# ramkp990/Truth_Recommendation_GNN

Hardware: NVIDIA B200
Metric: message-passing edges/s (train step) (higher is better)
Workload: dtype f32

## Files before the change

### include/trg_b200.h

```cpp
#ifndef TRG_B200_H
#define TRG_B200_H

#include <stddef.h>
#include <stdint.h>

#ifdef __cplusplus
extern "C" {
#endif

#define TRG_ABI_VERSION 4

enum { TRG_F32 = 0, TRG_BF16 = 1, TRG_F8E4M3 = 2  };
enum {
  TRG_OK = 0,
  TRG_E_ARG = 1,
  TRG_E_WORKSPACE = 2,
  TRG_E_CUDA = 3,
  TRG_E_UNSUPPORTED = 4
};

int trg_abi_version(void);
const char* trg_last_error(void);
int64_t trg_launch_count(void);

size_t trg_csr_workspace_bytes(int64_t n_edges, int64_t n_key);
int trg_csr_build(const int64_t* other, const int64_t* key, int64_t n_edges, int64_t n_key,
                  int32_t* rowptr , int32_t* col , int32_t* eid ,
                  void* workspace, size_t workspace_bytes, void* stream);

size_t trg_select_range_workspace_bytes(int64_t n);
int trg_select_range(const int64_t* key, const int64_t* other, int64_t n, int64_t lo, int64_t hi,
                     int64_t capacity, int64_t pad_key, int64_t pad_other,
                     int64_t* key_out , int64_t* other_out ,
                     int32_t* count_out , void* workspace, size_t workspace_bytes, void* stream);

typedef struct {
  const int32_t* vrowptr;
  const int32_t* vinfo;
  int64_t n_vrows;
  const int32_t* long_rows;
  const int32_t* long_ptr;
  int64_t n_long;
  float* partial;
} trg_long_rows;

int trg_sage_agg_fwd(const int32_t* rowptr, const int32_t* col, const void* x_src,
                     int64_t n_dst, int32_t feat, int dtype,
                     void* mean_out , float* inv_deg_out ,
                     const trg_long_rows* long_rows , void* stream);

int trg_sage_agg_bwd(const int32_t* rowptr_t, const int32_t* col_t, const float* inv_deg,
                     const void* g_mean, int64_t n_src, int32_t feat, int dtype,
                     void* g_src_out , int out_dtype, int accumulate,
                     const void* relu_of, const trg_long_rows* long_rows ,
                     void* stream);

int trg_gather_wsum(const int32_t* rowptr, const int32_t* col, const int32_t* eid,
                    const float* coef, const float* scale, const void* x,
                    int64_t n_rows, int32_t feat, int dtype, void* out, int out_dtype, int accumulate,
                    const void* relu_of, const trg_long_rows* long_rows , void* stream);

int trg_rows_finish(const void* in, int in_dtype, const float* row_scale, const void* add,
                    const void* relu_of, int64_t n_rows, int32_t feat, int dtype, void* out, void* stream);

int trg_peer_reduce_rows(const void* const* parts, int32_t n_peers, int64_t row0, int in_dtype,
                         const float* row_scale, const void* add, const void* relu_of, int64_t n_rows,
                         int32_t feat, int dtype, void* out, int32_t ctas_per_sm, void* stream);

size_t trg_edge_bce_workspace_bytes(int64_t n_users);
int trg_edge_bce_fwd(const int32_t* rowptr_u, const int32_t* col_p, const int32_t* eid,
                     const int64_t* neg_p, const void* u, const void* p,
                     int64_t n_users, int64_t n_edges, int32_t hidden, int dtype,
                     const float* wbar , float* loss_out,
                     float* c_pos, float* c_neg, void* g_u,
                     void* workspace, size_t workspace_bytes, void* stream);

int trg_edge_anchor_loss(const int32_t* rowptr, const int32_t* col, const int32_t* eid,
                         const void* anchor, const void* gathered, int64_t n_rows,
                         int64_t n_edges_scale, int32_t hidden, int dtype, int label,
                         const float* wbar, float* loss_out, float* coef_out, void* g_anchor,
                         int accumulate, int relu_gate, void* workspace, size_t workspace_bytes,
// ... 64 lines not shown
```

### truth_recommendation_gnn_b200/_lib.py

```python
from __future__ import annotations

import ctypes
import os

import torch

_HERE = os.path.dirname(os.path.abspath(__file__))
LIB_PATH = os.path.join(_HERE, "lib", "libtrg_b200.so")

TRG_F32, TRG_BF16, TRG_F8E4M3 = 0, 1, 2
ABI_VERSION = 4

_vp, _i64, _i32, _sz, _int = ctypes.c_void_p, ctypes.c_int64, ctypes.c_int32, ctypes.c_size_t, ctypes.c_int


class TrgProjTerm(ctypes.Structure):
    _fields_ = [("a", _vp), ("w", _vp), ("k", _i32), ("alpha", ctypes.c_float)]


class TrgLongRows(ctypes.Structure):
    _fields_ = [("vrowptr", _vp), ("vinfo", _vp), ("n_vrows", _i64), ("long_rows", _vp), ("long_ptr", _vp),
                ("n_long", _i64), ("partial", _vp)]


class TrgProjBwdTerm(ctypes.Structure):
    _fields_ = [("w", _vp), ("k", _i32), ("alpha", ctypes.c_float), ("row_scale", _vp), ("d_a", _vp)]


class TrgProjDwTerm(ctypes.Structure):
    _fields_ = [("a", _vp), ("k", _i32), ("alpha", ctypes.c_float), ("d_w", _vp)]


SIGNATURES = {
    "trg_abi_version": (_int, []),
    "trg_last_error": (ctypes.c_char_p, []),
    "trg_launch_count": (_i64, []),
    "trg_csr_workspace_bytes": (_sz, [_i64, _i64]),
    "trg_csr_build": (_int, [_vp, _vp, _i64, _i64, _vp, _vp, _vp, _vp, _sz, _vp]),
    "trg_select_range_workspace_bytes": (_sz, [_i64]),
    "trg_select_range": (_int, [_vp, _vp, _i64, _i64, _i64, _i64, _i64, _i64, _vp, _vp, _vp, _vp, _sz, _vp]),
    "trg_sage_agg_fwd": (_int, [_vp, _vp, _vp, _i64, _i32, _int, _vp, _vp, ctypes.POINTER(TrgLongRows), _vp]),
    "trg_sage_agg_bwd": (_int, [_vp, _vp, _vp, _vp, _i64, _i32, _int, _vp, _int, _int, _vp,
                                ctypes.POINTER(TrgLongRows), _vp]),
    "trg_gather_wsum": (_int, [_vp, _vp, _vp, _vp, _vp, _vp, _i64, _i32, _int, _vp, _int, _int, _vp,
                               ctypes.POINTER(TrgLongRows), _vp]),
    "trg_rows_finish": (_int, [_vp, _int, _vp, _vp, _vp, _i64, _i32, _int, _vp, _vp]),
    "trg_peer_reduce_rows": (_int, [_vp, _i32, _i64, _int, _vp, _vp, _vp, _i64, _i32, _int, _vp, _i32, _vp]),
    "trg_edge_bce_workspace_bytes": (_sz, [_i64]),
    "trg_edge_bce_fwd": (_int, [_vp, _vp, _vp, _vp, _vp, _vp, _i64, _i64, _i32, _int, _vp, _vp,
                                _vp, _vp, _vp, _vp, _sz, _vp]),
    "trg_edge_anchor_loss": (_int, [_vp, _vp, _vp, _vp, _vp, _i64, _i64, _i32, _int, _int, _vp, _vp, _vp,
                                    _vp, _int, _int, _vp, _sz, _vp]),
    "trg_sage_proj_workspace_bytes": (_sz, [_i32, _i32, _int]),
    "trg_sage_proj_fwd": (_int, [ctypes.POINTER(TrgProjTerm), _i32, _vp, _i64, _i32, _int, _int, _vp,
                                 _vp, _sz, _vp]),
    "trg_sage_proj_bwd_input": (_int, [_vp, ctypes.POINTER(TrgProjBwdTerm), _i32, _i64, _i32, _int,
                                       _vp, _sz, _vp]),
    "trg_sage_proj_dw_workspace_bytes": (_sz, []),
    "trg_sage_proj_bwd_weight": (_int, [_vp, ctypes.POINTER(TrgProjDwTerm), _i32, _vp, _i64, _i32, _int,
                                        _vp, _sz, _vp]),
    "trg_score_topk_workspace_bytes": (_sz, [_i64, _i64, _i32, _i32]),
    "trg_score_topk": (_int, [_vp, _vp, _i64, _i64, _i32, _int, _i32, _i64, _vp, _vp, _vp, _sz, _vp]),
    "trg_score_topk_excluding": (_int, [_vp, _vp, _i64, _i64, _i32, _int, _i32, _i64, _vp, _vp, _vp, _vp, _vp,
                                        _vp, _sz, _vp]),
    "trg_topk_merge": (_int, [_vp, _vp, _i64, _i32, _i32, _i32, _vp, _vp, _vp]),
    "trg_rescore_topk_workspace_bytes": (_sz, [_i64, _i32]),
    "trg_rescore_topk": (_int, [_vp, _vp, _i64, _i64, _i32, _int, _vp, _i32, _i64, _i32, _vp, _vp, _vp, _sz,
                                _vp]),
}

_lib = None


class TrgError(RuntimeError):
    pass


def load():
    global _lib
    if _lib is None:
        if not os.path.exists(LIB_PATH):
            raise TrgError(
                f"{LIB_PATH} is missing: build it with `python -m truth_recommendation_gnn_b200.build` "
                "(nvcc, sm_100a). There is no CPU or PyTorch fallback for the hot path.")
        lib = ctypes.CDLL(LIB_PATH)
        for name, (res, args) in SIGNATURES.items():
            fn = getattr(lib, name)
            fn.restype, fn.argtypes = res, args
        if lib.trg_abi_version() != ABI_VERSION:
            raise TrgError("libtrg_b200.so ABI version mismatch; rebuild")
        _lib = lib
# ... 68 lines not shown
```

### truth_recommendation_gnn_b200/csrc/csr_build.cu

```cuda
#include <algorithm>
#include <cstdio>

#include "common.cuh"

namespace trg {
namespace {

constexpr int kThreads = 256;
constexpr int kItems = 16;
constexpr int kTile = kThreads * kItems;
constexpr int kWarps = kThreads / 32;
constexpr int kRadix = 256;

template <int NWARPS>
__device__ __forceinline__ int block_exclusive_scan(int v, int* warp_sums, int& total) {
  const int lane = threadIdx.x & 31, w = threadIdx.x >> 5;
  int inc = v;
#pragma unroll
  for (int o = 1; o < 32; o <<= 1) {
    int t = __shfl_up_sync(0xffffffffu, inc, o);
    if (lane >= o) inc += t;
  }
  if (lane == 31) warp_sums[w] = inc;
  __syncthreads();
// ... 19 lines not shown
  for (int i = 0; i < kItems; ++i) {
    int64_t idx = base + (int64_t)i * kThreads + threadIdx.x;
    if (idx < n) s += in[idx];
  }
  int total;
  block_exclusive_scan<kWarps>(s, warp_sums, total);
  if (threadIdx.x == 0) tile_sums[blockIdx.x] = total;
}

__global__ void __launch_bounds__(1024) scan_tile_offsets(int* __restrict__ tile_sums, int n_tiles) {
  __shared__ int warp_sums[32];
  int carry = 0;
  for (int base = 0; base < n_tiles; base += 1024) {
    int idx = base + threadIdx.x;
    int v = idx < n_tiles ? tile_sums[idx] : 0;
    int total;
    int ex = block_exclusive_scan<32>(v, warp_sums, total);
    if (idx < n_tiles) tile_sums[idx] = carry + ex;
    carry += total;
  }
}

__global__ void __launch_bounds__(kThreads) scan_apply(const int* in, int* out, int64_t n,
                                                       const int* __restrict__ tile_offsets) {
  __shared__ int warp_sums[kWarps];
  const int64_t base = (int64_t)blockIdx.x * kTile + (int64_t)threadIdx.x * kItems;
  int v[kItems];
  int s = 0;
#pragma unroll
  for (int i = 0; i < kItems; ++i) {
    v[i] = (base + i < n) ? in[base + i] : 0;
    s += v[i];
  }
  int total;
  int run = block_exclusive_scan<kWarps>(s, warp_sums, total) + tile_offsets[blockIdx.x];
#pragma unroll
  for (int i = 0; i < kItems; ++i) {
    if (base + i < n) out[base + i] = run;
    run += v[i];
  }
}

int exclusive_scan(const int* in, int* out, int64_t n, int* tile_sums, cudaStream_t st) {
  if (n <= 0) return TRG_OK;
  const int n_tiles = (int)ceil_div<int64_t>(n, kTile);
  scan_tile_sums<<<n_tiles, kThreads, 0, st>>>(in, n, tile_sums);
  scan_tile_offsets<<<1, 1024, 0, st>>>(tile_sums, n_tiles);
  scan_apply<<<n_tiles, kThreads, 0, st>>>(in, out, n, tile_sums);
  count_launch(3);
  TRG_LAUNCH_OK();
  return TRG_OK;
}

__global__ void __launch_bounds__(kThreads) count_keys(const long long* __restrict__ key, int64_t n,
                                                       long long n_key, int* __restrict__ deg) {
  int64_t i = (int64_t)blockIdx.x * blockDim.x + threadIdx.x;
  const int64_t stride = (int64_t)gridDim.x * blockDim.x;
  for (; i < n; i += stride) {
    const long long k = ldg_stream(key + i);
    if ((unsigned long long)k >= (unsigned long long)n_key) {
      printf("trg_csr_build: key %lld at edge %lld is outside [0, %lld)\n", k, (long long)i, n_key);
      __trap();
    }
    atomicAdd(&deg[(int)k], 1);
  }
}


__global__ void __launch_bounds__(kThreads) select_count(const long long* __restrict__ key, int64_t n,
                                                         long long lo, long long hi, int* __restrict__ tile_counts) {
  __shared__ int warp_sums[kWarps];
  const int64_t base = (int64_t)blockIdx.x * kTile;
  int c = 0;
#pragma unroll
  for (int i = 0; i < kItems; ++i) {
    const int64_t idx = base + (int64_t)i * kThreads + threadIdx.x;
    if (idx < n) {
      const long long k = ldg_stream(key + idx);
      c += (k >= lo && k < hi) ? 1 : 0;
    }
  }
  int total;
  block_exclusive_scan<kWarps>(c, warp_sums, total);
  if (threadIdx.x == 0) tile_counts[blockIdx.x] = total;
}

__global__ void __launch_bounds__(1024) select_offsets(int* __restrict__ tile_counts, int n_tiles,
                                                       long long capacity, int* __restrict__ count_out) {
  __shared__ int warp_sums[32];
  int carry = 0;
  for (int base = 0; base < n_tiles; base += 1024) {
    const int idx = base + threadIdx.x;
    const int v = idx < n_tiles ? tile_counts[idx] : 0;
    int total;
    const int ex = block_exclusive_scan<32>(v, warp_sums, total);
    if (idx < n_tiles) tile_counts[idx] = carry + ex;
    carry += total;
  }
  if (threadIdx.x == 0) {
    *count_out = carry;
    if ((long long)carry > capacity) {
      printf("trg_select_range: %d selected entries exceed the capacity %lld (negatives far from uniform? pass a larger "
             "capacity)\n", carry, capacity);
      __trap();
    }
  }
}

__global__ void __launch_bounds__(kThreads)
    select_scatter(const long long* __restrict__ key, const long long* __restrict__ other, int64_t n, long long lo,
                   long long hi, const int* __restrict__ tile_offsets, const int* __restrict__ count,
                   long long capacity, long long pad_key, long long pad_other, long long* __restrict__ key_out,
                   long long* __restrict__ other_out) {
  __shared__ int wtot[kWarps];
  const int lane = threadIdx.x & 31, w = threadIdx.x >> 5;
  const int64_t wbase = (int64_t)blockIdx.x * kTile + (int64_t)w * (kItems * 32);
  long long kv[kItems];
  unsigned sel[kItems];
  int mine = 0;
#pragma unroll
  for (int r = 0; r < kItems; ++r) {
    const int64_t idx = wbase + r * 32 + lane;
    kv[r] = idx < n ? ldg_stream(key + idx) : lo - 1;
    const bool in = kv[r] >= lo && kv[r] < hi;
    sel[r] = __ballot_sync(0xffffffffu, in);
    mine += __popc(sel[r]);
  }
  if (lane == 0) wtot[w] = mine;
  __syncthreads();
  int run = tile_offsets[blockIdx.x];
  for (int i = 0; i < w; ++i) run += wtot[i];
#pragma unroll
  for (int r = 0; r < kItems; ++r) {
    if ((sel[r] >> lane) & 1u) {
      const int dest = run + __popc(sel[r] & ((1u << lane) - 1u));
      if (dest < capacity) {
        key_out[dest] = kv[r] - lo;
        other_out[dest] = ldg_stream(other + wbase + r * 32 + lane);
      }
    }
    run += __popc(sel[r]);
  }
  const long long cnt = *count;
  for (long long i = cnt + (long long)blockIdx.x * kThreads + threadIdx.x; i < capacity;
       i += (long long)gridDim.x * kThreads) {
    key_out[i] = pad_key;
    other_out[i] = pad_other;
  }
}

__device__ __forceinline__ uint2 ldg_pair(const uint2* p) {
  uint2 r;
  asm volatile("ld.global.nc.L1::no_allocate.v2.u32 {%0,%1}, [%2];" : "=r"(r.x), "=r"(r.y) : "l"(p));
  return r;
}
template <bool FIRST>
__device__ __forceinline__ uint32_t load_key(const void* keys, int64_t idx) {
  if (FIRST) return (uint32_t)ldg_stream(reinterpret_cast<const long long*>(keys) + idx);
  return ldg_pair(reinterpret_cast<const uint2*>(keys) + idx).x;
}

template <bool FIRST>
__global__ void __launch_bounds__(kThreads) radix_hist(const void* __restrict__ keys, int64_t n,
                                                       int shift, int* __restrict__ hist,
                                                       int n_ctas) {
  __shared__ int h[kRadix];
  h[threadIdx.x] = 0;
  __syncthreads();
  const int64_t base = (int64_t)blockIdx.x * kTile;
#pragma unroll
  for (int i = 0; i < kItems; ++i) {
    int64_t idx = base + (int64_t)i * kThreads + threadIdx.x;
    if (idx < n) atomicAdd(&h[(load_key<FIRST>(keys, idx) >> shift) & (kRadix - 1)], 1);
  }
  __syncthreads();
  hist[(int64_t)threadIdx.x * n_ctas + blockIdx.x] = h[threadIdx.x];
}

template <bool FIRST, bool LAST>
__global__ void __launch_bounds__(kThreads)
    radix_scatter(const void* __restrict__ keys_in, int64_t n, int shift, const int* __restrict__ gbase,
                  int n_ctas, uint2* __restrict__ pairs_out, uint32_t* __restrict__ vals_out) {
  __shared__ int wcnt[kWarps][kRadix];
  __shared__ int sbase[kRadix];
  const int lane = threadIdx.x & 31, w = threadIdx.x >> 5;
#pragma unroll
  for (int i = 0; i < kWarps; ++i) wcnt[i][threadIdx.x] = 0;
  const int64_t wbase = (int64_t)blockIdx.x * kTile + (int64_t)w * (kItems * 32);

  uint32_t key[kItems], val[kItems];
#pragma unroll
  for (int r = 0; r < kItems; ++r) {
    int64_t idx = wbase + r * 32 + lane;
    bool valid = idx < n;
    if (FIRST) {
      key[r] = valid ? load_key<true>(keys_in, idx) : 0u;
      val[r] = (uint32_t)idx;
    } else {
      const uint2 kv = valid ? ldg_pair(reinterpret_cast<const uint2*>(keys_in) + idx) : make_uint2(0u, 0u);
      key[r] = kv.x;
      val[r] = kv.y;
    }
  }
  __syncthreads();

  int rank[kItems];
#pragma unroll
  for (int r = 0; r < kItems; ++r) {
    const bool valid = wbase + r * 32 + lane < n;
    const int d = valid ? (int)((key[r] >> shift) & (kRadix - 1)) : kRadix;
    const unsigned peers = __match_any_sync(0xffffffffu, d);
    const int prev = valid ? wcnt[w][d] : 0;
    __syncwarp();
    if (valid && lane == __ffs(peers) - 1) wcnt[w][d] = prev + __popc(peers);
    __syncwarp();
    rank[r] = prev + __popc(peers & ((1u << lane) - 1u));
  }
  __syncthreads();
  {
    int run = 0;
#pragma unroll
    for (int i = 0; i < kWarps; ++i) {
      int t = wcnt[i][threadIdx.x];
      wcnt[i][threadIdx.x] = run;
      run += t;
    }
    sbase[threadIdx.x] = gbase[(int64_t)threadIdx.x * n_ctas + blockIdx.x];
  }
  __syncthreads();
#pragma unroll
  for (int r = 0; r < kItems; ++r) {
    if (wbase + r * 32 + lane < n) {
      const int d = (int)((key[r] >> shift) & (kRadix - 1));
      const int dest = sbase[d] + wcnt[w][d] + rank[r];
      if (LAST)
        vals_out[dest] = val[r];
      else
        pairs_out[dest] = make_uint2(key[r], val[r]);
    }
  }
}

__global__ void __launch_bounds__(kThreads) gather_col(const long long* __restrict__ other,
                                                       const int* __restrict__ eid, int64_t n,
                                                       int* __restrict__ col) {
  int64_t i = (int64_t)blockIdx.x * blockDim.x + threadIdx.x;
  const int64_t stride = (int64_t)gridDim.x * blockDim.x;
  for (; i < n; i += stride) col[i] = (int)other[ldg_stream(eid + i)];
}

int num_passes(int64_t n_key) {
  int bits = 1;
  while (bits < 32 && ((int64_t)1 << bits) < n_key) ++bits;
  return (bits + 7) / 8;
}

struct Workspace {
  uint2* pairs[2];
  uint32_t* vals;
  int *hist, *tile_sums;
  size_t bytes;
};

Workspace carve(void* ws, int64_t e, int64_t n_key) {
  Workspace w;
  const size_t ebytes = align_up((size_t)(e > 0 ? e : 1) * 4, 256);
  const int64_t n_ctas = ceil_div<int64_t>(e > 0 ? e : 1, kTile);
  const size_t hist_bytes = align_up((size_t)kRadix * n_ctas * 4, 256);
  const int64_t scan_len = (int64_t)kRadix * n_ctas > n_key + 1 ? (int64_t)kRadix * n_ctas : n_key + 1;
  const size_t sums_bytes = align_up((size_t)ceil_div<int64_t>(scan_len, kTile) * 4 + 4, 256);
  char* p = reinterpret_cast<char*>(ws);
  w.pairs[0] = (uint2*)p; p += 2 * ebytes;
  w.pairs[1] = (uint2*)p; p += 2 * ebytes;
  w.vals = (uint32_t*)p; p += ebytes;
  w.hist = (int*)p; p += hist_bytes;
  w.tile_sums = (int*)p; p += sums_bytes;
  w.bytes = (size_t)(p - reinterpret_cast<char*>(ws));
  return w;
}

}
}

using namespace trg;

extern "C" size_t trg_csr_workspace_bytes(int64_t n_edges, int64_t n_key) {
  if (n_edges < 0 || n_key < 0) return 0;
  return carve(nullptr, n_edges, n_key).bytes;
}

extern "C" int trg_csr_build(const int64_t* other, const int64_t* key, int64_t e, int64_t n_key,
                             int32_t* rowptr, int32_t* col, int32_t* eid, void* workspace,
                             size_t workspace_bytes, void* stream) {
  cudaStream_t st = reinterpret_cast<cudaStream_t>(stream);
  TRG_CHECK_ARG(e >= 0 && n_key >= 0, "trg_csr_build: negative size");
  TRG_CHECK_ARG(e < ((int64_t)1 << 31) && n_key < ((int64_t)1 << 31) - 1,
                "trg_csr_build: n_edges=%lld / n_key=%lld exceed int32 CSR range", (long long)e,
                (long long)n_key);
  TRG_CHECK_ARG(rowptr != nullptr, "trg_csr_build: rowptr is NULL");
  TRG_CHECK_ARG(e == 0 || (key != nullptr && (col == nullptr || other != nullptr)),
                "trg_csr_build: NULL edge arrays with n_edges > 0");
  TRG_CHECK_ARG(e == 0 || n_key > 0, "trg_csr_build: edges present but n_key == 0");
  Workspace w = carve(workspace, e, n_key);
  if (workspace == nullptr || workspace_bytes < w.bytes) {
    set_error("trg_csr_build: workspace %zu < required %zu", workspace_bytes, w.bytes);
    return TRG_E_WORKSPACE;
  }
  TRG_CUDA(cudaMemsetAsync(rowptr, 0, (size_t)(n_key + 1) * sizeof(int32_t), st));
  if (e == 0) return TRG_OK;

  {
    int grid = (int)std::min<int64_t>(ceil_div<int64_t>(e, kThreads), (int64_t)kNumSMs * 16);
    count_keys<<<grid, kThreads, 0, st>>>((const long long*)key, e, (long long)n_key, rowptr);
    count_launch();
    TRG_LAUNCH_OK();
    int rc = exclusive_scan(rowptr, rowptr, n_key + 1, w.tile_sums, st);
    if (rc) return rc;
  }
  if (col == nullptr && eid == nullptr) return TRG_OK;

  const int passes = num_passes(n_key);
  const int n_ctas = (int)ceil_div<int64_t>(e, kTile);
  const void* kin = key;
  const uint32_t* vin = nullptr;
  for (int p = 0; p < passes; ++p) {
    const bool first = p == 0, last = p == passes - 1;
    const int shift = 8 * p;
    uint2* kout = w.pairs[p & 1];
    uint32_t* vout = eid ? (uint32_t*)eid : w.vals;
    if (first)
      radix_hist<true><<<n_ctas, kThreads, 0, st>>>(kin, e, shift, w.hist, n_ctas);
    else
      radix_hist<false><<<n_ctas, kThreads, 0, st>>>(kin, e, shift, w.hist, n_ctas);
    count_launch();
    TRG_LAUNCH_OK();
    int rc = exclusive_scan(w.hist, w.hist, (int64_t)kRadix * n_ctas, w.tile_sums, st);
    if (rc) return rc;
    if (first && last)
      radix_scatter<true, true><<<n_ctas, kThreads, 0, st>>>(kin, e, shift, w.hist, n_ctas, kout, vout);
    else if (first)
      radix_scatter<true, false><<<n_ctas, kThreads, 0, st>>>(kin, e, shift, w.hist, n_ctas, kout, vout);
    else if (last)
      radix_scatter<false, true><<<n_ctas, kThreads, 0, st>>>(kin, e, shift, w.hist, n_ctas, kout, vout);
    else
      radix_scatter<false, false><<<n_ctas, kThreads, 0, st>>>(kin, e, shift, w.hist, n_ctas, kout, vout);
    count_launch();
    TRG_LAUNCH_OK();
    kin = kout;
    vin = vout;
  }
  if (col != nullptr) {
    int grid = (int)std::min<int64_t>(ceil_div<int64_t>(e, kThreads), (int64_t)kNumSMs * 16);
    gather_col<<<grid, kThreads, 0, st>>>((const long long*)other, (const int*)vin, e, col);
    count_launch();
    TRG_LAUNCH_OK();
  }
  return TRG_OK;
}

extern "C" size_t trg_select_range_workspace_bytes(int64_t n) {
  if (n < 0) return 0;
  return align_up((size_t)(ceil_div<int64_t>(n > 0 ? n : 1, kTile) + 1) * 4, 256);
}

extern "C" int trg_select_range(const int64_t* key, const int64_t* other, int64_t n, int64_t lo, int64_t hi,
                                int64_t capacity, int64_t pad_key, int64_t pad_other, int64_t* key_out,
                                int64_t* other_out, int32_t* count_out, void* workspace, size_t workspace_bytes,
                                void* stream) {
  cudaStream_t st = reinterpret_cast<cudaStream_t>(stream);
  TRG_CHECK_ARG(n >= 0 && capacity >= 0 && lo <= hi, "trg_select_range: bad sizes");
  TRG_CHECK_ARG(n < ((int64_t)1 << 31) && capacity < ((int64_t)1 << 31), "trg_select_range: sizes exceed int32 range");
  TRG_CHECK_ARG(count_out && (capacity == 0 || (key_out && other_out)), "trg_select_range: NULL outputs");
  TRG_CHECK_ARG(n == 0 || (key && other), "trg_select_range: NULL inputs with n > 0");
  if (workspace == nullptr || workspace_bytes < trg_select_range_workspace_bytes(n)) {
    set_error("trg_select_range: workspace %zu < required %zu", workspace_bytes, trg_select_range_workspace_bytes(n));
    return TRG_E_WORKSPACE;
  }
  int* tile_counts = reinterpret_cast<int*>(workspace);
  const int n_tiles = (int)ceil_div<int64_t>(n > 0 ? n : 1, kTile);
  select_count<<<n_tiles, kThreads, 0, st>>>((const long long*)key, n, lo, hi, tile_counts);
  select_offsets<<<1, 1024, 0, st>>>(tile_counts, n_tiles, capacity, count_out);
  select_scatter<<<n_tiles, kThreads, 0, st>>>((const long long*)key, (const long long*)other, n, lo, hi, tile_counts,
                                               count_out, capacity, pad_key, pad_other, (long long*)key_out,
                                               (long long*)other_out);
  count_launch(3);
  TRG_LAUNCH_OK();
  return TRG_OK;
}
```

### truth_recommendation_gnn_b200/fused_step.py

```python
from __future__ import annotations

import torch

from . import _lib
from .functional import (edge_anchor_loss, gather_wsum, link_structure, sage_agg_bwd, sage_agg_fwd,
                         sage_proj_bwd_input, sage_proj_bwd_weight, sage_proj_fwd)
from .graph import CSR, build_csr, relation_graph
from .nn import REL_DIRECT, REL_ENGAGE, REL_SOCIAL, StackedWeightedRGCN, WeightedRGCN


def _layers(model):
    if type(model) is StackedWeightedRGCN:
        return list(model.layers)
    if type(model) is WeightedRGCN:
        return [model]
    return None


def model_eligible(model) -> bool:
    layers = _layers(model)
    if layers is None or not torch.is_grad_enabled():
        return False
    if any(conv.lin_l.bias is None for l in layers for conv in (l.msg_direct, l.msg_social, l.post_update)):
        return False
    return all(p.requires_grad for p in model.parameters())


def eligible(model, x_dict) -> bool:
    if not model_eligible(model):
        return False
    xu, xp = x_dict["user"], x_dict["post"]
    return xu.is_cuda and xp.is_cuda and not xu.requires_grad and not xp.requires_grad and xu.dtype == xp.dtype


def _agg(rel, x):
    want_inv = rel.inv_deg is None
    mean, inv_deg = sage_agg_fwd(rel.fwd, x, want_inv_deg=want_inv)
    if want_inv:
        rel.inv_deg = inv_deg
    return mean


@torch.no_grad()
def loss_and_grads(model, x_dict, edge_index_dict, train_edge_index, interaction_type_tensor, num_users,
                   neg_p, neg_ready=None):
    layers = _layers(model)
    if layers is None:
        raise _lib.TrgError("loss_and_grads: model must be WeightedRGCN or StackedWeightedRGCN")
    hu, hp = x_dict["user"].contiguous(), x_dict["post"].contiguous()
    n_u, n_p = hu.size(0), hp.size(0)
    rel_d = relation_graph(edge_index_dict[REL_DIRECT], n_p, n_u)
    rel_s = relation_graph(edge_index_dict[REL_SOCIAL], n_u, n_u)
    rel_e = relation_graph(edge_index_dict[REL_ENGAGE], n_u, n_p)

    saved = []
    for layer in layers:
        layer.materialize(hu.size(-1), hp.size(-1))
        mean_d, mean_s, mean_e = _agg(rel_d, hp), _agg(rel_s, hu), _agg(rel_e, hu)
        ug, pg = layer.user_gemm(), layer.post_gemm()
        hu_n = sage_proj_fwd(ug.terms(mean_d, mean_s, hu), ug.bias, True)
        hp_n = sage_proj_fwd(pg.terms(mean_e, hp), pg.bias, True)
        saved.append((hu, hp, mean_d, mean_s, mean_e, ug, pg))
        hu, hp = hu_n, hp_n

    ls = link_structure(train_edge_index, interaction_type_tensor, num_users, n_p)
    if neg_ready is not None:
        torch.cuda.current_stream().wait_event(neg_ready)
    if neg_p.dtype != torch.int64 or neg_p.numel() != ls.n_edges:
        raise _lib.TrgError("neg_p must be int64 with one entry per positive edge (train_gnn.py:272)")
    if getattr(ls, "eid_long", None) is None:
        ls.eid_long = ls.by_user.eid.long()
    bu = ls.by_user
    col_neg64 = neg_p.index_select(0, ls.eid_long)
    neg_by_post = build_csr(ls.user_of_u, col_neg64, n_p, n_u, validate=False, per_step=True)
    neg_by_user = CSR(bu.rowptr, col_neg64.int(), bu.eid, bu.n_rows, bu.n_cols)
    l_pos, c_pos, dz_u = edge_anchor_loss(bu, hu, hp, ls.n_edges, 1, ls.wbar, True, None, coef_in_csr_order=True)
    l_neg, c_neg, dz_u = edge_anchor_loss(neg_by_user, hu, hp, ls.n_edges, 0, ls.wbar, True, dz_u,
                                          relu_gate=True, coef_in_csr_order=True)
    dz_p = gather_wsum(ls.by_post_u, c_pos, hu)
    gather_wsum(neg_by_post, c_neg, hu, out=dz_p, accumulate=True, relu_of=hp)
    del col_neg64
    loss = (l_pos + l_neg).reshape(())
    del neg_by_user, neg_by_post, c_pos, c_neg, hu, hp

    for li in range(len(layers) - 1, -1, -1):
        hu_in, hp_in, mean_d, mean_s, mean_e, ug, pg = saved.pop()
        dw_u, db_u = sage_proj_bwd_weight(dz_u, ug.dw_terms(mean_d, mean_s, hu_in), True)
        dw_p, db_p = sage_proj_bwd_weight(dz_p, pg.dw_terms(mean_e, hp_in), True)
        del mean_d, mean_s, mean_e
        layers[li].accumulate_grads(dw_u, db_u, dw_p, db_p)
        if li == 0:
            break
        g_md, g_ms, g_hu = sage_proj_bwd_input(dz_u, ug.dx_terms(rel_d.inv_deg, rel_s.inv_deg, None))
        g_me, g_hp = sage_proj_bwd_input(dz_p, pg.dx_terms(rel_e.inv_deg, None))
        del dz_u, dz_p
        sage_agg_bwd(rel_s.bwd, None, g_ms, out=g_hu, accumulate=True)
        sage_agg_bwd(rel_e.bwd, None, g_me, out=g_hu, accumulate=True, relu_of=hu_in)
        sage_agg_bwd(rel_d.bwd, None, g_md, out=g_hp, accumulate=True, relu_of=hp_in)
        dz_u, dz_p = g_hu, g_hp
    return loss
```

### truth_recommendation_gnn_b200/graph.py

```python
from __future__ import annotations

from collections import OrderedDict
from dataclasses import dataclass

import torch

from . import _lib


LONG_ROW_THRESHOLD = 1024


@dataclass
class LongRows:
    vrowptr: torch.Tensor
    vinfo: torch.Tensor
    long_rows: torch.Tensor
    long_ptr: torch.Tensor
    n_slots: int


@dataclass
class CSR:
    rowptr: torch.Tensor
# ... 15 lines not shown

def _split_long_rows(csr: "CSR", t: int):
    if csr.n_rows == 0 or csr.n_edges <= t:
        return None
    rp = csr.rowptr.long()
    deg = rp[1:] - rp[:-1]
    if int(deg.max()) <= t:
        return None
    is_long = deg > t
    counts = torch.where(is_long, (deg + t - 1) // t, torch.ones_like(deg))
    n_vrows = int(counts.sum())
    orig = torch.repeat_interleave(torch.arange(csr.n_rows, device=rp.device), counts)
    vstart = torch.cumsum(counts, 0) - counts
    k = torch.arange(n_vrows, device=rp.device) - vstart[orig]
    vrowptr = torch.empty(n_vrows + 1, dtype=torch.int32, device=rp.device)
    vrowptr[:-1] = (rp[:-1][orig] + k * t).int()
    vrowptr[-1] = csr.n_edges
    part = is_long[orig]
    slot = torch.cumsum(part.long(), 0) - 1
    vinfo = torch.where(part, -(slot + 1), orig).int()
    long_ids = is_long.nonzero().flatten()
    lp = torch.zeros(long_ids.numel() + 1, dtype=torch.long, device=rp.device)
    lp[1:] = torch.cumsum(counts[long_ids], 0)
    return LongRows(vrowptr, vinfo, long_ids.int(), lp.int(), int(lp[-1]))


def build_csr(other: torch.Tensor, key: torch.Tensor, n_key: int, n_other: int,
              validate: bool = True, per_step: bool = False) -> CSR:
    lib = _lib.load()
    if key.dtype != torch.int64 or other.dtype != torch.int64:
        raise TypeError("edge_index must be int64 (torch.long), as in the reference")
    key = key.contiguous()
    other = other.contiguous()
    e = int(key.numel())
    dev = key.device
    if validate and e > 0:
        lo_k, hi_k = int(key.min()), int(key.max())
        lo_o, hi_o = int(other.min()), int(other.max())
        if lo_k < 0 or hi_k >= n_key or lo_o < 0 or hi_o >= n_other:
            raise IndexError(f"edge_index out of range: key in [{lo_k},{hi_k}] vs {n_key}, "
                             f"other in [{lo_o},{hi_o}] vs {n_other}")
    rowptr = torch.empty(n_key + 1, dtype=torch.int32, device=dev)
    col = torch.empty(e, dtype=torch.int32, device=dev)
    eid = torch.empty(e, dtype=torch.int32, device=dev)
    ws_bytes = int(lib.trg_csr_workspace_bytes(e, n_key))
    ws = torch.empty(ws_bytes, dtype=torch.uint8, device=dev)
    _lib.call("trg_csr_build", e * 80 + 8 * (n_key + 1), lib.trg_csr_build,
              _lib.ptr(other) if e else None, _lib.ptr(key) if e else None, e, n_key, _lib.ptr(rowptr),
              _lib.ptr(col) if e else None, _lib.ptr(eid) if e else None, _lib.ptr(ws), ws_bytes,
              _lib.stream())
    return CSR(rowptr, col, eid, n_key, n_other, False if per_step else None)


class RelationGraph:

    def __init__(self, edge_index: torch.Tensor, n_src: int, n_dst: int):
        if edge_index.dim() != 2 or edge_index.size(0) != 2:
            raise ValueError("edge_index must have shape [2, E]")
        self.edge_index = edge_index
        self.n_src, self.n_dst = int(n_src), int(n_dst)
        self._fwd = None
        self._bwd = None
        self.inv_deg = None

    @property
    def fwd(self) -> CSR:
        if self._fwd is None:
            ei = self.edge_index
            self._fwd = build_csr(ei[0], ei[1], self.n_dst, self.n_src)
        return self._fwd

    @property
    def bwd(self) -> CSR:
        if self._bwd is None:
            ei = self.edge_index
            self._bwd = build_csr(ei[1], ei[0], self.n_src, self.n_dst, validate=self._fwd is None)
        return self._bwd


class PushRelation:

    def __init__(self, rel: RelationGraph, inv_deg: torch.Tensor):
        self.rel = rel
        self.inv_deg = inv_deg


class GraphCache:

    def __init__(self, capacity: int = 32):
        self.capacity = capacity
        self._d: OrderedDict = OrderedDict()

    def get(self, edge_index: torch.Tensor, n_src: int, n_dst: int) -> RelationGraph:
        key = (edge_index.data_ptr(), tuple(edge_index.shape), edge_index._version,
               int(n_src), int(n_dst), str(edge_index.device))
        g = self._d.get(key)
        if g is None:
            g = RelationGraph(edge_index, n_src, n_dst)
            self._d[key] = g
            while len(self._d) > self.capacity:
                self._d.popitem(last=False)
        else:
            self._d.move_to_end(key)
        return g

    def clear(self):
# ... 13 lines not shown
```

Before: 2.986 billion.

## Switch CSR radix sort to onesweep with decoupled lookback and fused gather

Replaces the per-pass histogram, scan and scatter radix sort with a single up-front histogram for all digit passes and a onesweep scatter that uses decoupled look-back prefix sums. The scatter is staged through shared memory for more coalesced writes. The 'other' column is carried through the sort instead of being gathered at the end. A new gather-variant entry point fuses the negative-sample index_select into the histogram kernel, and the per-step negative CSR build uses it. The goal is fewer kernel launches and less global traffic per step, at the cost of spin-waiting look-back and a larger status workspace.

```diff
diff --git a/include/trg_b200.h b/include/trg_b200.h
--- a/include/trg_b200.h
+++ b/include/trg_b200.h
@@ -27,6 +27,10 @@
 int trg_csr_build(const int64_t* other, const int64_t* key, int64_t n_edges, int64_t n_key,
                   int32_t* rowptr , int32_t* col , int32_t* eid ,
                   void* workspace, size_t workspace_bytes, void* stream);
+int trg_csr_build_gather(const int64_t* other , const int64_t* key, const int32_t* key_index ,
+                         int64_t n_edges, int64_t n_key, int32_t* key_out ,
+                         int32_t* rowptr , int32_t* col , int32_t* eid ,
+                         void* workspace, size_t workspace_bytes, void* stream);
 
 size_t trg_select_range_workspace_bytes(int64_t n);
 int trg_select_range(const int64_t* key, const int64_t* other, int64_t n, int64_t lo, int64_t hi,
diff --git a/truth_recommendation_gnn_b200/_lib.py b/truth_recommendation_gnn_b200/_lib.py
--- a/truth_recommendation_gnn_b200/_lib.py
+++ b/truth_recommendation_gnn_b200/_lib.py
@@ -37,6 +37,7 @@
     "trg_launch_count": (_i64, []),
     "trg_csr_workspace_bytes": (_sz, [_i64, _i64]),
     "trg_csr_build": (_int, [_vp, _vp, _i64, _i64, _vp, _vp, _vp, _vp, _sz, _vp]),
+    "trg_csr_build_gather": (_int, [_vp, _vp, _vp, _i64, _i64, _vp, _vp, _vp, _vp, _vp, _sz, _vp]),
     "trg_select_range_workspace_bytes": (_sz, [_i64]),
     "trg_select_range": (_int, [_vp, _vp, _i64, _i64, _i64, _i64, _i64, _i64, _vp, _vp, _vp, _vp, _sz, _vp]),
     "trg_sage_agg_fwd": (_int, [_vp, _vp, _vp, _i64, _i32, _int, _vp, _vp, ctypes.POINTER(TrgLongRows), _vp]),
diff --git a/truth_recommendation_gnn_b200/csrc/csr_build.cu b/truth_recommendation_gnn_b200/csrc/csr_build.cu
--- a/truth_recommendation_gnn_b200/csrc/csr_build.cu
+++ b/truth_recommendation_gnn_b200/csrc/csr_build.cu
@@ -95,20 +95,59 @@
   return TRG_OK;
 }
 
-__global__ void __launch_bounds__(kThreads) count_keys(const long long* __restrict__ key, int64_t n,
-                                                       long long n_key, int* __restrict__ deg) {
-  int64_t i = (int64_t)blockIdx.x * blockDim.x + threadIdx.x;
-  const int64_t stride = (int64_t)gridDim.x * blockDim.x;
-  for (; i < n; i += stride) {
-    const long long k = ldg_stream(key + i);
-    if ((unsigned long long)k >= (unsigned long long)n_key) {
-      printf("trg_csr_build: key %lld at edge %lld is outside [0, %lld)\n", k, (long long)i, n_key);
-      __trap();
-    }
-    atomicAdd(&deg[(int)k], 1);
-  }
-}
-
+constexpr int kMaxPasses = 4;
+
+template <bool GATHER>
+__global__ void __launch_bounds__(kThreads)
+    key_hist(const long long* __restrict__ key, const int* __restrict__ key_index, int64_t n, long long n_key,
+             int passes, int* __restrict__ deg, int* __restrict__ ghist, int* __restrict__ key_out) {
+  __shared__ int h[kMaxPasses][kRadix];
+#pragma unroll
+  for (int p = 0; p < kMaxPasses; ++p) h[p][threadIdx.x] = 0;
+  __syncthreads();
+  const int64_t n_tiles = ceil_div<int64_t>(n, kTile);
+  for (int64_t t = blockIdx.x; t < n_tiles; t += gridDim.x) {
+    const int64_t base = t * kTile + threadIdx.x;
+    long long k[kItems];
+    if (GATHER) {
+      int src[kItems];
+#pragma unroll
+      for (int i = 0; i < kItems; ++i) {
+        const int64_t idx = base + (int64_t)i * kThreads;
+        src[i] = idx < n ? ldg_stream(key_index + idx) : 0;
+      }
+#pragma unroll
+      for (int i = 0; i < kItems; ++i)
+        k[i] = base + (int64_t)i * kThreads < n ? ldg_stream(key + src[i]) : 0;
+    } else {
+#pragma unroll
+      for (int i = 0; i < kItems; ++i) {
+        const int64_t idx = base + (int64_t)i * kThreads;
+        k[i] = idx < n ? ldg_stream(key + idx) : 0;
+      }
+    }
+#pragma unroll
+    for (int i = 0; i < kItems; ++i) {
+      const int64_t idx = base + (int64_t)i * kThreads;
+      if (idx >= n) continue;
+      if ((unsigned long long)k[i] >= (unsigned long long)n_key) {
+        printf("trg_csr_build: key %lld at edge %lld is outside [0, %lld)\n", k[i], (long long)idx, n_key);
+        __trap();
+      }
+      atomicAdd(&deg[(int)k[i]], 1);
+      if (GATHER) key_out[idx] = (int)k[i];
+#pragma unroll
+      for (int p = 0; p < kMaxPasses; ++p)
+        if (p < passes) atomicAdd(&h[p][((uint32_t)k[i] >> (8 * p)) & (kRadix - 1)], 1);
+    }
+  }
+  __syncthreads();
+#pragma unroll
+  for (int p = 0; p < kMaxPasses; ++p) {
+    const int v = h[p][threadIdx.x];
+    if (p < passes && v) atomicAdd(&ghist[p * kRadix + threadIdx.x], v);
+  }
+}
 
 __global__ void __launch_bounds__(kThreads) select_count(const long long* __restrict__ key, int64_t n,
                                                          long long lo, long long hi, int* __restrict__ tile_counts) {
@@ -192,60 +231,69 @@
   }
 }
 
+constexpr unsigned long long kAgg = 1ull << 32, kPrefix = 2ull << 32;
+constexpr int kLookback = 16;
+enum KeySrc { kKey64 = 0, kKey32 = 1, kPairs = 2 };
+
 __device__ __forceinline__ uint2 ldg_pair(const uint2* p) {
   uint2 r;
   asm volatile("ld.global.nc.L1::no_allocate.v2.u32 {%0,%1}, [%2];" : "=r"(r.x), "=r"(r.y) : "l"(p));
   return r;
 }
-template <bool FIRST>
-__device__ __forceinline__ uint32_t load_key(const void* keys, int64_t idx) {
-  if (FIRST) return (uint32_t)ldg_stream(reinterpret_cast<const long long*>(keys) + idx);
-  return ldg_pair(reinterpret_cast<const uint2*>(keys) + idx).x;
-}
-
-template <bool FIRST>
-__global__ void __launch_bounds__(kThreads) radix_hist(const void* __restrict__ keys, int64_t n,
-                                                       int shift, int* __restrict__ hist,
-                                                       int n_ctas) {
-  __shared__ int h[kRadix];
-  h[threadIdx.x] = 0;
-  __syncthreads();
-  const int64_t base = (int64_t)blockIdx.x * kTile;
-#pragma unroll
-  for (int i = 0; i < kItems; ++i) {
-    int64_t idx = base + (int64_t)i * kThreads + threadIdx.x;
-    if (idx < n) atomicAdd(&h[(load_key<FIRST>(keys, idx) >> shift) & (kRadix - 1)], 1);
-  }
-  __syncthreads();
-  hist[(int64_t)threadIdx.x * n_ctas + blockIdx.x] = h[threadIdx.x];
-}
-
-template <bool FIRST, bool LAST>
+__device__ __forceinline__ unsigned long long ld_status(const unsigned long long* p) {
+  unsigned long long r;
+  asm volatile("ld.relaxed.gpu.global.u64 %0, [%1];" : "=l"(r) : "l"(p) : "memory");
+  return r;
+}
+__device__ __forceinline__ void st_status(unsigned long long* p, unsigned long long v) {
+  asm volatile("st.relaxed.gpu.global.u64 [%0], %1;" ::"l"(p), "l"(v) : "memory");
+}
+
+template <int SRC, bool OTHER, bool LAST>
 __global__ void __launch_bounds__(kThreads)
-    radix_scatter(const void* __restrict__ keys_in, int64_t n, int shift, const int* __restrict__ gbase,
-                  int n_ctas, uint2* __restrict__ pairs_out, uint32_t* __restrict__ vals_out) {
-  __shared__ int wcnt[kWarps][kRadix];
-  __shared__ int sbase[kRadix];
+    onesweep(const void* __restrict__ keys_in, const void* __restrict__ other_in, int64_t n, int shift,
+             const int* __restrict__ ghist, unsigned long long* __restrict__ status, int* __restrict__ tile_counter,
+             uint2* __restrict__ pairs_out, uint32_t* __restrict__ other_out, int* __restrict__ eid_out,
+             int* __restrict__ col_out) {
+  extern __shared__ uint32_t stage[];
+  uint32_t* skey = stage;
+  uint32_t* spos = stage + kTile;
+  uint32_t* soth = stage + 2 * kTile;
+  int(*wcnt)[kRadix] = reinterpret_cast<int(*)[kRadix]>(stage);
+  __shared__ int sdelta[kRadix];
+  __shared__ int lbase[kRadix];
+  __shared__ int warp_sums[kWarps];
+  __shared__ int s_tile;
+
   const int lane = threadIdx.x & 31, w = threadIdx.x >> 5;
+  if (threadIdx.x == 0) s_tile = atomicAdd(tile_counter, 1);
 #pragma unroll
   for (int i = 0; i < kWarps; ++i) wcnt[i][threadIdx.x] = 0;
-  const int64_t wbase = (int64_t)blockIdx.x * kTile + (int64_t)w * (kItems * 32);
-
-  uint32_t key[kItems], val[kItems];
+  __syncthreads();
+  const int tile = s_tile;
+  const int64_t wbase = (int64_t)tile * kTile + (int64_t)w * (kItems * 32);
+
+  uint32_t key[kItems], pos[kItems], oth[kItems];
 #pragma unroll
   for (int r = 0; r < kItems; ++r) {
-    int64_t idx = wbase + r * 32 + lane;
-    bool valid = idx < n;
-    if (FIRST) {
-      key[r] = valid ? load_key<true>(keys_in, idx) : 0u;
-      val[r] = (uint32_t)idx;
+    const int64_t idx = wbase + r * 32 + lane;
+    const bool valid = idx < n;
+    if (SRC == kKey64) {
+      key[r] = valid ? (uint32_t)ldg_stream(reinterpret_cast<const long long*>(keys_in) + idx) : 0u;
+    } else if (SRC == kKey32) {
+      key[r] = valid ? (uint32_t)ldg_stream(reinterpret_cast<const int*>(keys_in) + idx) : 0u;
     } else {
       const uint2 kv = valid ? ldg_pair(reinterpret_cast<const uint2*>(keys_in) + idx) : make_uint2(0u, 0u);
       key[r] = kv.x;
-      val[r] = kv.y;
-    }
-  }
-  __syncthreads();
+      pos[r] = kv.y;
+    }
+    if (OTHER) {
+      if (SRC == kPairs)
+        oth[r] = valid ? (uint32_t)ldg_stream(reinterpret_cast<const int*>(other_in) + idx) : 0u;
+      else
+        oth[r] = valid ? (uint32_t)ldg_stream(reinterpret_cast<const long long*>(other_in) + idx) : 0u;
+    }
+  }
 
   int rank[kItems];
 #pragma unroll
@@ -260,36 +308,106 @@
     rank[r] = prev + __popc(peers & ((1u << lane) - 1u));
   }
   __syncthreads();
-  {
-    int run = 0;
-#pragma unroll
-    for (int i = 0; i < kWarps; ++i) {
-      int t = wcnt[i][threadIdx.x];
-      wcnt[i][threadIdx.x] = run;
-      run += t;
-    }
-    sbase[threadIdx.x] = gbase[(int64_t)threadIdx.x * n_ctas + blockIdx.x];
-  }
-  __syncthreads();
+
+  int cnt = 0;
+#pragma unroll
+  for (int i = 0; i < kWarps; ++i) {
+    const int t = wcnt[i][threadIdx.x];
+    wcnt[i][threadIdx.x] = cnt;
+    cnt += t;
+  }
+  unsigned long long* my_status = status + (int64_t)tile * kRadix + threadIdx.x;
+  st_status(my_status, (tile == 0 ? kPrefix : kAgg) | (unsigned)cnt);
+
+  int total;
+  const int lb = block_exclusive_scan<kWarps>(cnt, warp_sums, total);
+  lbase[threadIdx.x] = lb;
+  __syncthreads();
+
+  int* slot = rank;
 #pragma unroll
   for (int r = 0; r < kItems; ++r) {
-    if (wbase + r * 32 + lane < n) {
-      const int d = (int)((key[r] >> shift) & (kRadix - 1));
-      const int dest = sbase[d] + wcnt[w][d] + rank[r];
-      if (LAST)
-        vals_out[dest] = val[r];
-      else
-        pairs_out[dest] = make_uint2(key[r], val[r]);
-    }
-  }
-}
-
-__global__ void __launch_bounds__(kThreads) gather_col(const long long* __restrict__ other,
-                                                       const int* __restrict__ eid, int64_t n,
-                                                       int* __restrict__ col) {
-  int64_t i = (int64_t)blockIdx.x * blockDim.x + threadIdx.x;
-  const int64_t stride = (int64_t)gridDim.x * blockDim.x;
-  for (; i < n; i += stride) col[i] = (int)other[ldg_stream(eid + i)];
+    const int d = (int)((key[r] >> shift) & (kRadix - 1));
+    slot[r] = wbase + r * 32 + lane < n ? lbase[d] + wcnt[w][d] + rank[r] : -1;
+  }
+  __syncthreads();
+#pragma unroll
+  for (int r = 0; r < kItems; ++r) {
+    if (slot[r] >= 0) {
+      skey[slot[r]] = key[r];
+      spos[slot[r]] = SRC == kPairs ? pos[r] : (uint32_t)(wbase + r * 32 + lane);
+      if (OTHER) soth[slot[r]] = oth[r];
+    }
+  }
+
+  const int gb = block_exclusive_scan<kWarps>(ghist[threadIdx.x], warp_sums, total);
+  int earlier = 0;
+  for (int64_t j = (int64_t)tile - 1; j >= 0;) {
+    unsigned long long sw[kLookback];
+#pragma unroll
+    for (int k = 0; k < kLookback; ++k)
+      sw[k] = j - k >= 0 ? ld_status(status + (j - k) * kRadix + threadIdx.x) : kPrefix;
+    int k = 0;
+    bool done = false;
+#pragma unroll
+    for (int q = 0; q < kLookback; ++q) {
+      if (sw[q] == 0) break;
+      earlier += (int)(uint32_t)sw[q];
+      ++k;
+      if (sw[q] & kPrefix) {
+        done = true;
+        break;
+      }
+    }
+    if (done) break;
+    j -= k;
+  }
+  if (tile > 0) st_status(my_status, kPrefix | (unsigned)(earlier + cnt));
+  sdelta[threadIdx.x] = gb + earlier - lb;
+  __syncthreads();
+
+  const int64_t rest = n - (int64_t)tile * kTile;
+  const int tile_n = rest < kTile ? (int)rest : kTile;
+  for (int s = threadIdx.x; s < tile_n; s += kThreads) {
+    const int dest = sdelta[(skey[s] >> shift) & (kRadix - 1)] + s;
+    if (LAST) {
+      if (eid_out != nullptr) eid_out[dest] = (int)spos[s];
+      if (OTHER) col_out[dest] = (int)soth[s];
+    } else {
+      pairs_out[dest] = make_uint2(skey[s], spos[s]);
+      if (OTHER) other_out[dest] = soth[s];
+    }
+  }
+}
+
+constexpr int stage_bytes(bool other) { return (other ? 3 : 2) * kTile * (int)sizeof(uint32_t); }
+static_assert(kWarps * kRadix <= 2 * kTile, "per-warp digit counters must fit in the staging buffer");
+static_assert(kThreads == kRadix, "one thread per digit in the look-back");
+
+template <int SRC, bool OTHER, bool LAST>
+int launch_onesweep(int n_tiles, cudaStream_t st, const void* keys_in, const void* other_in, int64_t n, int shift,
+                    const int* ghist, unsigned long long* status, int* tile_counter, uint2* pairs_out,
+                    uint32_t* other_out, int* eid_out, int* col_out) {
+  static SmemAttrState attr;
+  auto kernel = onesweep<SRC, OTHER, LAST>;
+  TRG_CUDA(ensure_dyn_smem(kernel, stage_bytes(OTHER), attr));
+  kernel<<<n_tiles, kThreads, stage_bytes(OTHER), st>>>(keys_in, other_in, n, shift, ghist, status, tile_counter,
+                                                        pairs_out, other_out, eid_out, col_out);
+  count_launch();
+  TRG_LAUNCH_OK();
+  return TRG_OK;
+}
+
+template <int SRC>
+int launch_pass(bool other, bool last, int n_tiles, cudaStream_t st, const void* keys_in, const void* other_in,
+                int64_t n, int shift, const int* ghist, unsigned long long* status, int* tile_counter,
+                uint2* pairs_out, uint32_t* other_out, int* eid_out, int* col_out) {
+#define TRG_PASS(O, L)                                                                                              \
+  launch_onesweep<SRC, O, L>(n_tiles, st, keys_in, other_in, n, shift, ghist, status, tile_counter, pairs_out, \
+                             other_out, eid_out, col_out)
+  if (other) return last ? TRG_PASS(true, true) : TRG_PASS(true, false);
+  return last ? TRG_PASS(false, true) : TRG_PASS(false, false);
+#undef TRG_PASS
 }
 
 int num_passes(int64_t n_key) {
@@ -300,50 +418,39 @@
 
 struct Workspace {
   uint2* pairs[2];
-  uint32_t* vals;
-  int *hist, *tile_sums;
+  uint32_t* other[2];
+  int* ghist;
+  int* tile_counter;
+  unsigned long long* status;
+  size_t zero_bytes;
+  int* tile_sums;
   size_t bytes;
 };
 
 Workspace carve(void* ws, int64_t e, int64_t n_key) {
   Workspace w;
   const size_t ebytes = align_up((size_t)(e > 0 ? e : 1) * 4, 256);
-  const int64_t n_ctas = ceil_div<int64_t>(e > 0 ? e : 1, kTile);
-  const size_t hist_bytes = align_up((size_t)kRadix * n_ctas * 4, 256);
-  const int64_t scan_len = (int64_t)kRadix * n_ctas > n_key + 1 ? (int64_t)kRadix * n_ctas : n_key + 1;
-  const size_t sums_bytes = align_up((size_t)ceil_div<int64_t>(scan_len, kTile) * 4 + 4, 256);
+  const int64_t n_tiles = ceil_div<int64_t>(e > 0 ? e : 1, kTile);
+  const size_t status_bytes = (size_t)num_passes(n_key) * n_tiles * kRadix * sizeof(unsigned long long);
+  const size_t sums_bytes = align_up((size_t)ceil_div<int64_t>(n_key + 1, kTile) * 4 + 4, 256);
   char* p = reinterpret_cast<char*>(ws);
   w.pairs[0] = (uint2*)p; p += 2 * ebytes;
   w.pairs[1] = (uint2*)p; p += 2 * ebytes;
-  w.vals = (uint32_t*)p; p += ebytes;
-  w.hist = (int*)p; p += hist_bytes;
+  w.other[0] = (uint32_t*)p; p += ebytes;
+  w.other[1] = (uint32_t*)p; p += ebytes;
+  char* z = p;
+  w.ghist = (int*)p; p += kMaxPasses * kRadix * 4;
+  w.tile_counter = (int*)p; p += 256;
+  w.status = (unsigned long long*)p; p += align_up(status_bytes, 256);
+  w.zero_bytes = (size_t)(p - z);
   w.tile_sums = (int*)p; p += sums_bytes;
   w.bytes = (size_t)(p - reinterpret_cast<char*>(ws));
   return w;
 }
 
-}
-}
-
-using namespace trg;
-
-extern "C" size_t trg_csr_workspace_bytes(int64_t n_edges, int64_t n_key) {
-  if (n_edges < 0 || n_key < 0) return 0;
-  return carve(nullptr, n_edges, n_key).bytes;
-}
-
-extern "C" int trg_csr_build(const int64_t* other, const int64_t* key, int64_t e, int64_t n_key,
-                             int32_t* rowptr, int32_t* col, int32_t* eid, void* workspace,
-                             size_t workspace_bytes, void* stream) {
-  cudaStream_t st = reinterpret_cast<cudaStream_t>(stream);
-  TRG_CHECK_ARG(e >= 0 && n_key >= 0, "trg_csr_build: negative size");
-  TRG_CHECK_ARG(e < ((int64_t)1 << 31) && n_key < ((int64_t)1 << 31) - 1,
-                "trg_csr_build: n_edges=%lld / n_key=%lld exceed int32 CSR range", (long long)e,
-                (long long)n_key);
-  TRG_CHECK_ARG(rowptr != nullptr, "trg_csr_build: rowptr is NULL");
-  TRG_CHECK_ARG(e == 0 || (key != nullptr && (col == nullptr || other != nullptr)),
-                "trg_csr_build: NULL edge arrays with n_edges > 0");
-  TRG_CHECK_ARG(e == 0 || n_key > 0, "trg_csr_build: edges present but n_key == 0");
+int csr_build(const int64_t* other, const int64_t* key, const int32_t* key_index, int32_t* key_out, int64_t e,
+              int64_t n_key, int32_t* rowptr, int32_t* col, int32_t* eid, void* workspace, size_t workspace_bytes,
+              cudaStream_t st) {
   Workspace w = carve(workspace, e, n_key);
   if (workspace == nullptr || workspace_bytes < w.bytes) {
     set_error("trg_csr_build: workspace %zu < required %zu", workspace_bytes, w.bytes);
@@ -352,53 +459,86 @@
   TRG_CUDA(cudaMemsetAsync(rowptr, 0, (size_t)(n_key + 1) * sizeof(int32_t), st));
   if (e == 0) return TRG_OK;
 
+  const bool sort = col != nullptr || eid != nullptr;
+  const int passes = sort ? num_passes(n_key) : 0;
+  const int n_tiles = (int)ceil_div<int64_t>(e, kTile);
+  if (sort) TRG_CUDA(cudaMemsetAsync(w.ghist, 0, w.zero_bytes, st));
   {
-    int grid = (int)std::min<int64_t>(ceil_div<int64_t>(e, kThreads), (int64_t)kNumSMs * 16);
-    count_keys<<<grid, kThreads, 0, st>>>((const long long*)key, e, (long long)n_key, rowptr);
+    const int grid = std::min(n_tiles, kNumSMs * 8);
+    if (key_index)
+      key_hist<true><<<grid, kThreads, 0, st>>>((const long long*)key, key_index, e, (long long)n_key, passes,
+                                                rowptr, w.ghist, key_out);
+    else
+      key_hist<false><<<grid, kThreads, 0, st>>>((const long long*)key, nullptr, e, (long long)n_key, passes,
+                                                 rowptr, w.ghist, nullptr);
     count_launch();
     TRG_LAUNCH_OK();
     int rc = exclusive_scan(rowptr, rowptr, n_key + 1, w.tile_sums, st);
     if (rc) return rc;
   }
-  if (col == nullptr && eid == nullptr) return TRG_OK;
-
-  const int passes = num_passes(n_key);
-  const int n_ctas = (int)ceil_div<int64_t>(e, kTile);
-  const void* kin = key;
-  const uint32_t* vin = nullptr;
+  if (!sort) return TRG_OK;
+
+  const bool want_other = col != nullptr;
+  const void* kin = key_index ? (const void*)key_out : (const void*)key;
+  const void* oin = other;
   for (int p = 0; p < passes; ++p) {
-    const bool first = p == 0, last = p == passes - 1;
-    const int shift = 8 * p;
+    const bool last = p == passes - 1;
+    unsigned long long* status = w.status + (int64_t)p * n_tiles * kRadix;
     uint2* kout = w.pairs[p & 1];
-    uint32_t* vout = eid ? (uint32_t*)eid : w.vals;
-    if (first)
-      radix_hist<true><<<n_ctas, kThreads, 0, st>>>(kin, e, shift, w.hist, n_ctas);
+    uint32_t* oout = w.other[p & 1];
+    int rc;
+    if (p > 0)
+      rc = launch_pass<kPairs>(want_other, last, n_tiles, st, kin, oin, e, 8 * p, w.ghist + p * kRadix, status,
+                               w.tile_counter + p, kout, oout, eid, col);
+    else if (key_index)
+      rc = launch_pass<kKey32>(want_other, last, n_tiles, st, kin, oin, e, 0, w.ghist, status, w.tile_counter, kout,
+                               oout, eid, col);
     else
-      radix_hist<false><<<n_ctas, kThreads, 0, st>>>(kin, e, shift, w.hist, n_ctas);
-    count_launch();
-    TRG_LAUNCH_OK();
-    int rc = exclusive_scan(w.hist, w.hist, (int64_t)kRadix * n_ctas, w.tile_sums, st);
+      rc = launch_pass<kKey64>(want_other, last, n_tiles, st, kin, oin, e, 0, w.ghist, status, w.tile_counter, kout,
+                               oout, eid, col);
     if (rc) return rc;
-    if (first && last)
-      radix_scatter<true, true><<<n_ctas, kThreads, 0, st>>>(kin, e, shift, w.hist, n_ctas, kout, vout);
-    else if (first)
-      radix_scatter<true, false><<<n_ctas, kThreads, 0, st>>>(kin, e, shift, w.hist, n_ctas, kout, vout);
-    else if (last)
-      radix_scatter<false, true><<<n_ctas, kThreads, 0, st>>>(kin, e, shift, w.hist, n_ctas, kout, vout);
-    else
-      radix_scatter<false, false><<<n_ctas, kThreads, 0, st>>>(kin, e, shift, w.hist, n_ctas, kout, vout);
-    count_launch();
-    TRG_LAUNCH_OK();
     kin = kout;
-    vin = vout;
-  }
-  if (col != nullptr) {
-    int grid = (int)std::min<int64_t>(ceil_div<int64_t>(e, kThreads), (int64_t)kNumSMs * 16);
-    gather_col<<<grid, kThreads, 0, st>>>((const long long*)other, (const int*)vin, e, col);
-    count_launch();
-    TRG_LAUNCH_OK();
+    oin = oout;
   }
   return TRG_OK;
+}
+
+}
+}
+
+using namespace trg;
+
+extern "C" size_t trg_csr_workspace_bytes(int64_t n_edges, int64_t n_key) {
+  if (n_edges < 0 || n_key < 0) return 0;
+  return carve(nullptr, n_edges, n_key).bytes;
+}
+
+#define TRG_CSR_CHECK_SIZES(name)                                                                          \
+  TRG_CHECK_ARG(e >= 0 && n_key >= 0, name ": negative size");                                             \
+  TRG_CHECK_ARG(e < ((int64_t)1 << 31) && n_key < ((int64_t)1 << 31) - 1,                                  \
+                name ": n_edges=%lld / n_key=%lld exceed int32 CSR range", (long long)e, (long long)n_key); \
+  TRG_CHECK_ARG(rowptr != nullptr, name ": rowptr is NULL");                                               \
+  TRG_CHECK_ARG(e == 0 || n_key > 0, name ": edges present but n_key == 0")
+
+extern "C" int trg_csr_build(const int64_t* other, const int64_t* key, int64_t e, int64_t n_key,
+                             int32_t* rowptr, int32_t* col, int32_t* eid, void* workspace,
+                             size_t workspace_bytes, void* stream) {
+  TRG_CSR_CHECK_SIZES("trg_csr_build");
+  TRG_CHECK_ARG(e == 0 || (key != nullptr && (col == nullptr || other != nullptr)),
+                "trg_csr_build: NULL edge arrays with n_edges > 0");
+  return csr_build(other, key, nullptr, nullptr, e, n_key, rowptr, col, eid, workspace, workspace_bytes,
+                   reinterpret_cast<cudaStream_t>(stream));
+}
+
+extern "C" int trg_csr_build_gather(const int64_t* other, const int64_t* key, const int32_t* key_index,
+                                    int64_t e, int64_t n_key, int32_t* key_out, int32_t* rowptr, int32_t* col,
+                                    int32_t* eid, void* workspace, size_t workspace_bytes, void* stream) {
+  TRG_CSR_CHECK_SIZES("trg_csr_build_gather");
+  TRG_CHECK_ARG(e == 0 || (key != nullptr && key_index != nullptr && key_out != nullptr &&
+                           (col == nullptr || other != nullptr)),
+                "trg_csr_build_gather: NULL edge arrays with n_edges > 0");
+  return csr_build(other, key, key_index, key_out, e, n_key, rowptr, col, eid, workspace, workspace_bytes,
+                   reinterpret_cast<cudaStream_t>(stream));
 }
 
 extern "C" size_t trg_select_range_workspace_bytes(int64_t n) {
diff --git a/truth_recommendation_gnn_b200/fused_step.py b/truth_recommendation_gnn_b200/fused_step.py
--- a/truth_recommendation_gnn_b200/fused_step.py
+++ b/truth_recommendation_gnn_b200/fused_step.py
@@ -5,7 +5,7 @@
 from . import _lib
 from .functional import (edge_anchor_loss, gather_wsum, link_structure, sage_agg_bwd, sage_agg_fwd,
                          sage_proj_bwd_input, sage_proj_bwd_weight, sage_proj_fwd)
-from .graph import CSR, build_csr, relation_graph
+from .graph import CSR, build_csr_gather, relation_graph
 from .nn import REL_DIRECT, REL_ENGAGE, REL_SOCIAL, StackedWeightedRGCN, WeightedRGCN
 
 
@@ -68,18 +68,15 @@
         torch.cuda.current_stream().wait_event(neg_ready)
     if neg_p.dtype != torch.int64 or neg_p.numel() != ls.n_edges:
         raise _lib.TrgError("neg_p must be int64 with one entry per positive edge (train_gnn.py:272)")
-    if getattr(ls, "eid_long", None) is None:
-        ls.eid_long = ls.by_user.eid.long()
     bu = ls.by_user
-    col_neg64 = neg_p.index_select(0, ls.eid_long)
-    neg_by_post = build_csr(ls.user_of_u, col_neg64, n_p, n_u, validate=False, per_step=True)
-    neg_by_user = CSR(bu.rowptr, col_neg64.int(), bu.eid, bu.n_rows, bu.n_cols)
+    neg_by_post, col_neg = build_csr_gather(ls.user_of_u, neg_p, bu.eid, n_p, n_u)
+    neg_by_user = CSR(bu.rowptr, col_neg, bu.eid, bu.n_rows, bu.n_cols)
     l_pos, c_pos, dz_u = edge_anchor_loss(bu, hu, hp, ls.n_edges, 1, ls.wbar, True, None, coef_in_csr_order=True)
     l_neg, c_neg, dz_u = edge_anchor_loss(neg_by_user, hu, hp, ls.n_edges, 0, ls.wbar, True, dz_u,
                                           relu_gate=True, coef_in_csr_order=True)
     dz_p = gather_wsum(ls.by_post_u, c_pos, hu)
     gather_wsum(neg_by_post, c_neg, hu, out=dz_p, accumulate=True, relu_of=hp)
-    del col_neg64
+    del col_neg
     loss = (l_pos + l_neg).reshape(())
     del neg_by_user, neg_by_post, c_pos, c_neg, hu, hp
 
diff --git a/truth_recommendation_gnn_b200/graph.py b/truth_recommendation_gnn_b200/graph.py
--- a/truth_recommendation_gnn_b200/graph.py
+++ b/truth_recommendation_gnn_b200/graph.py
@@ -91,6 +91,29 @@
     return CSR(rowptr, col, eid, n_key, n_other, False if per_step else None)
 
 
+def build_csr_gather(other: torch.Tensor, key: torch.Tensor, key_index: torch.Tensor, n_key: int, n_other: int,
+                     per_step: bool = True):
+    lib = _lib.load()
+    if key.dtype != torch.int64 or other.dtype != torch.int64 or key_index.dtype != torch.int32:
+        raise TypeError("build_csr_gather: key / other must be int64 and key_index int32")
+    key, other, key_index = key.contiguous(), other.contiguous(), key_index.contiguous()
+    e = int(key_index.numel())
+    if other.numel() != e:
+        raise ValueError("build_csr_gather: other and key_index must have one entry per edge")
+    dev = key.device
+    rowptr = torch.empty(n_key + 1, dtype=torch.int32, device=dev)
+    key_out = torch.empty(e, dtype=torch.int32, device=dev)
+    col = torch.empty(e, dtype=torch.int32, device=dev)
+    eid = torch.empty(e, dtype=torch.int32, device=dev)
+    ws_bytes = int(lib.trg_csr_workspace_bytes(e, n_key))
+    ws = torch.empty(ws_bytes, dtype=torch.uint8, device=dev)
+    _lib.call("trg_csr_build", e * 84 + 8 * (n_key + 1), lib.trg_csr_build_gather,
+              _lib.ptr(other) if e else None, _lib.ptr(key) if e else None, _lib.ptr(key_index) if e else None,
+              e, n_key, _lib.ptr(key_out) if e else None, _lib.ptr(rowptr), _lib.ptr(col) if e else None,
+              _lib.ptr(eid) if e else None, _lib.ptr(ws), ws_bytes, _lib.stream())
+    return CSR(rowptr, col, eid, n_key, n_other, False if per_step else None), key_out
+
+
 class RelationGraph:
 
     def __init__(self, edge_index: torch.Tensor, n_src: int, n_dst: int):
```

Measured after the change: 2.999 billion, median of 6. Within noise of the previous version (+0.4%).
